# harmoniqs/DirectTrajOpt.jl

Hardware: NVIDIA B200
Metric: full NLP evals/sec (constraint+Jacobian+Hessian) (higher is better)
Workload: dtype f64

## Files before the change

directtrajopt.jl_b200/csrc/bilinear_persistent.cu:

```cuda
#include <stdlib.h>

#include "dto_internal.h"
#include "series_tables.cuh"
#include "bulk_copy.cuh"

namespace {

constexpr int kMaxDrives = 4;
constexpr int kMaxWarps = 12;

__device__ __forceinline__ void dmma(double& c0, double& c1, double a, double b) {
    asm("mma.sync.aligned.m8n8k4.row.col.f64.f64.f64.f64 {%0,%1}, {%2}, {%3}, {%0,%1};" : "+d"(c0), "+d"(c1) : "d"(a), "d"(b));
}

__device__ __forceinline__ double quad_sum(double v) {
    v += __shfl_xor_sync(0xffffffffu, v, 1);
    v += __shfl_xor_sync(0xffffffffu, v, 2);
    return v;
}
__device__ __forceinline__ double warp_max(double v) {
#pragma unroll
    for (int o = 16; o > 0; o >>= 1) v = fmax(v, __shfl_xor_sync(0xffffffffu, v, o));
    return v;
}
// ... 7 lines not shown
template <int MT, int NT, int MD>
__device__ __forceinline__ void mma_apply(double (&out)[MT][NT][2], const double (&v)[MD][NT][2], const double* __restrict__ M,
                                          int lane) {
    constexpr int n = 8 * NT;
    const int row8 = lane >> 2;
    const int d = (NT % 2 == 0) ? ((row8 & 1) << 3) : 0;
    const double* base = M + row8 * n + 2 * (lane & 3);
#pragma unroll
    for (int t = 0; t < NT; ++t) {
        const int off = 8 * t + ((t & 1) ? -d : d);
        double2 b[NT];
#pragma unroll
        for (int nt = 0; nt < NT; ++nt) b[nt] = *reinterpret_cast<const double2*>(base + 8 * nt * n + off);
#pragma unroll
        for (int nt = 0; nt < NT; ++nt)
#pragma unroll
            for (int mt = 0; mt < MT; ++mt) dmma(out[mt][nt][0], out[mt][nt][1], v[mt][t][0], b[nt].x);
#pragma unroll
        for (int nt = 0; nt < NT; ++nt)
#pragma unroll
            for (int mt = 0; mt < MT; ++mt) dmma(out[mt][nt][0], out[mt][nt][1], v[mt][t][1], b[nt].y);
    }
}

template <int MT, int NT>
__device__ __forceinline__ void frag_zero(double (&f)[MT][NT][2]) {
#pragma unroll
    for (int mt = 0; mt < MT; ++mt)
#pragma unroll
        for (int nt = 0; nt < NT; ++nt) f[mt][nt][0] = f[mt][nt][1] = 0.0;
}

enum { ROLE_FWD = 0, ROLE_EXP = 1, ROLE_ADJ = 2 };

template <int NT>
struct Ctx {
    const DProb* P;
    const DInt* I;
    const double* Z;
    const double* mu;
    double* g;
    double* jac;
    const double* Gs;
    double* Gu;
    double* vbuf;
    double* M3;
    double* S2;
    int lane, want_jac, want_hess;
    int jets;
    const double2* plan;
};

template <int NT>
__device__ __forceinline__ double build_generator(const Ctx<NT>& c, const double (&uu)[kMaxDrives], int m, bool need_norm = true) {
    constexpr int n = 8 * NT, nn = n * n;
    for (int p = c.lane; p < nn; p += 32) {
        double v = c.Gs[p];
#pragma unroll
        for (int i = 0; i < kMaxDrives; ++i)
            if (i < m) v = fma(uu[i], c.Gs[(1 + i) * nn + p], v);
        c.Gu[p] = v;
    }
    __syncwarp();
    if (!need_norm) return 0.0;
    double cmax = 0.0;
    for (int k = c.lane; k < n; k += 32) {
        double s1 = 0.0;
        for (int s = 0; s < n; ++s) s1 += fabs(c.Gu[sw<NT>(s, k)]);
        cmax = fmax(cmax, s1);
    }
    return warp_max(cmax);
}

template <int NT>
__device__ __forceinline__ Series interval_series(const Ctx<NT>& c, int b, int kk, double dt, const double (&uu)[kMaxDrives], int m) {
    if (c.plan != nullptr) {
        build_generator<NT>(c, uu, m, false);
        return choose_series(c.plan[(long long)b * c.P->nI + kk]);
    }
    return choose_series(fabs(dt) * build_generator<NT>(c, uu, m));
}

template <int NT>
__device__ __forceinline__ void adjoint_drive_products(const double* __restrict__ Gs, const double* __restrict__ avec,
                                                       double* __restrict__ ybuf, int m, int lane) {
    constexpr int n = 8 * NT, nn = n * n;
    if constexpr (n >= 32) {
        for (int s = lane; s < n; s += 32) {
            double y[kMaxDrives] = {0.0, 0.0, 0.0, 0.0};
            for (int k = 0; k < n; k += 2) {
                const double2 a2 = *reinterpret_cast<const double2*>(avec + k);
                const int p0 = sw<NT>(k, s), p1 = sw<NT>(k + 1, s);
#pragma unroll
                for (int i = 0; i < kMaxDrives; ++i)
                    if (i < m) {
                        y[i] = fma(Gs[(1 + i) * nn + p0], a2.x, y[i]);
                        y[i] = fma(Gs[(1 + i) * nn + p1], a2.y, y[i]);
                    }
            }
#pragma unroll
            for (int i = 0; i < kMaxDrives; ++i)
                if (i < m) ybuf[i * n + s] = y[i];
        }
    } else {
        constexpr int KS = 32 / n;
        constexpr int KL = n / KS;
        const int s = lane % n, part = lane / n;
        double y[kMaxDrives] = {0.0, 0.0, 0.0, 0.0};
        if (part < KS) {
#pragma unroll
            for (int kk = 0; kk < KL; kk += 2) {
                const int k = part * KL + kk;
                const double2 a2 = *reinterpret_cast<const double2*>(avec + k);
                const int p0 = sw<NT>(k, s), p1 = sw<NT>(k + 1, s);
#pragma unroll
                for (int i = 0; i < kMaxDrives; ++i)
                    if (i < m) {
                        y[i] = fma(Gs[(1 + i) * nn + p0], a2.x, y[i]);
                        y[i] = fma(Gs[(1 + i) * nn + p1], a2.y, y[i]);
                    }
            }
        }
#pragma unroll
        for (int i = 0; i < kMaxDrives; ++i)
            if (i < m) {
#pragma unroll
                for (int off = n; off < 32 && off < n * KS; off <<= 1) y[i] += __shfl_xor_sync(0xffffffffu, y[i], off);
                if (lane < n) ybuf[i * n + s] = y[i];
            }
    }
}

template <int NT, int MT>
__device__ __forceinline__ void role_forward(const Ctx<NT>& c, int b, int kk, const int (&src)[kMaxDrives][MT],
                                             const double (&coef)[kMaxDrives][MT]) {
    constexpr int n = 8 * NT, nn = n * n;
    const DProb& P = *c.P;
    const DInt& I = *c.I;
    const int m = I.m, z = P.z, lane = c.lane, q = lane & 3, row8 = lane >> 2;
    const double* zk = c.Z + (long long)b * P.n_vars_local + (long long)kk * z;
    const double* zk1 = zk + z;
    if (P.halo != nullptr && kk + 1 == P.nK - 1) zk1 = P.halo;
    const double dt = zk[P.dt_off];
    double uu[kMaxDrives];
#pragma unroll
    for (int i = 0; i < kMaxDrives; ++i) uu[i] = i < m ? zk[I.u_off + i] : 0.0;
    const Series ser = interval_series<NT>(c, b, kk, dt, uu, m);
    const long long mu_off = (long long)b * P.n_cons_local + I.row_off + (long long)kk * n;
    const bool deriv = c.want_jac || c.want_hess || c.jets == DTO_JETS_STORE;
    const double* Gu = c.Gu;

    double F[MT][NT][2], term[MT][NT][2];
    frag_zero(F);
    if (row8 == 0) {
#pragma unroll
        for (int nt = 0; nt < NT; ++nt) {
            F[0][nt][0] = zk[I.x_off + 8 * nt + 2 * q];
            F[0][nt][1] = zk[I.x_off + 8 * nt + 2 * q + 1];
        }
    }
    for (int st = 0; st < ser.stages; ++st) {
#pragma unroll
        for (int mt = 0; mt < MT; ++mt)
#pragma unroll
            for (int nt = 0; nt < NT; ++nt) {
                term[mt][nt][0] = F[mt][nt][0];
                term[mt][nt][1] = F[mt][nt][1];
            }
        for (int t = 1; t <= ser.terms; ++t) {
            const double cf = dt * ser.inv_stages * kInv[t];
            double nw[MT][NT][2];
            frag_zero(nw);
            mma_apply<MT, NT, MT>(nw, term, Gu, lane);
#pragma unroll
            for (int i = 0; i < kMaxDrives; ++i) {
                if (i < m && deriv) {
                    double tmp[1][NT][2];
                    frag_zero(tmp);
                    mma_apply<1, NT, MT>(tmp, term, c.Gs + (1 + i) * nn, lane);
#pragma unroll
                    for (int mt = 0; mt < MT; ++mt)
#pragma unroll
                        for (int nt = 0; nt < NT; ++nt) {
                            const double v0 = __shfl_sync(0xffffffffu, tmp[0][nt][0], src[i][mt]);
                            const double v1 = __shfl_sync(0xffffffffu, tmp[0][nt][1], src[i][mt]);
                            nw[mt][nt][0] = fma(coef[i][mt], v0, nw[mt][nt][0]);
                            nw[mt][nt][1] = fma(coef[i][mt], v1, nw[mt][nt][1]);
                        }
                }
            }
#pragma unroll
            for (int mt = 0; mt < MT; ++mt)
#pragma unroll
                for (int nt = 0; nt < NT; ++nt) {
                    term[mt][nt][0] = cf * nw[mt][nt][0];
                    term[mt][nt][1] = cf * nw[mt][nt][1];
                    F[mt][nt][0] += term[mt][nt][0];
                    F[mt][nt][1] += term[mt][nt][1];
                }
        }
    }
    double GF[1][NT][2];
    frag_zero(GF);
    mma_apply<1, NT, MT>(GF, F, Gu, lane);
    if (c.g != nullptr && row8 == 0) {
        double* gp = c.g + mu_off;
#pragma unroll
        for (int nt = 0; nt < NT; ++nt) {
            gp[8 * nt + 2 * q] = zk1[I.x_off + 8 * nt + 2 * q] - F[0][nt][0];
            gp[8 * nt + 2 * q + 1] = zk1[I.x_off + 8 * nt + 2 * q + 1] - F[0][nt][1];
        }
    }
    if (c.want_jac) {
        double* jp = c.jac + (long long)b * P.nnz_jac_local;
        const long long own_off = jac_own_off(P, kk, I.doff, n);
        const long long prev_off = jac_prev_off(P, kk + 1, I.doff);
        for (int e = lane; e < 2 * z * n; e += 32) {
            const int l = e / n, a = e % n;
            if (l < z) {
                if ((l >= I.x_off && l < I.x_off + n) || (l >= I.u_off && l < I.u_off + m) || l == P.dt_off) continue;
                jp[jac_col(P, kk, l) + own_off + a] = 0.0;
            } else {
                jp[jac_col(P, (kk + 1), (l - z)) + prev_off + a] = (l - z - I.x_off == a) ? 1.0 : 0.0;
            }
        }
        if (row8 >= 1 && row8 <= m) {
            double* col = jp + jac_col(P, kk, I.u_off + (row8 - 1)) + own_off;
#pragma unroll
            for (int nt = 0; nt < NT; ++nt) {
                col[8 * nt + 2 * q] = -F[0][nt][0];
                col[8 * nt + 2 * q + 1] = -F[0][nt][1];
            }
        }
        if (row8 == 0) {
            double* col = jp + jac_col(P, kk, P.dt_off) + own_off;
#pragma unroll
            for (int nt = 0; nt < NT; ++nt) {
                col[8 * nt + 2 * q] = -GF[0][nt][0];
                col[8 * nt + 2 * q + 1] = -GF[0][nt][1];
            }
        }
    }
    if (c.want_hess && c.jets == DTO_JETS_NONE) {
        const int np = m + 1;
        double* hpp = I.hs + ((long long)b * P.nI + kk) * I.hs_stride + (long long)np * n;
        double muf[NT][2];
#pragma unroll
        for (int nt = 0; nt < NT; ++nt) {
            muf[nt][0] = c.mu[mu_off + 8 * nt + 2 * q];
            muf[nt][1] = c.mu[mu_off + 8 * nt + 2 * q + 1];
        }
#pragma unroll
// ... 62 lines not shown
        double GGF[1][NT][2];
        frag_zero(GGF);
        mma_apply<1, NT, 1>(GGF, GF, Gu, lane);
        if (row8 == 0) {
            double* w = W + (long long)J2 * n;
#pragma unroll
            for (int nt = 0; nt < NT; ++nt) {
                w[8 * nt + 2 * q] = GGF[0][nt][0];
                w[8 * nt + 2 * q + 1] = GGF[0][nt][1];
            }
        }
        if (row8 >= 1 && row8 <= m) {
            double* w = W + (long long)(J2 + 1 + m + (row8 - 1)) * n;
#pragma unroll
            for (int nt = 0; nt < NT; ++nt) {
                w[8 * nt + 2 * q] = GF[0][nt][0];
                w[8 * nt + 2 * q + 1] = GF[0][nt][1];
            }
        }
#pragma unroll
        for (int i = 0; i < kMaxDrives; ++i) {
            if (i < m) {
                double GiF[1][NT][2];
                frag_zero(GiF);
                mma_apply<1, NT, MT>(GiF, F, c.Gs + (1 + i) * nn, lane);
                if (row8 == 0) {
                    double* w = W + (long long)(J2 + 1 + i) * n;
#pragma unroll
                    for (int nt = 0; nt < NT; ++nt) {
                        w[8 * nt + 2 * q] = GiF[0][nt][0];
                        w[8 * nt + 2 * q + 1] = GiF[0][nt][1];
                    }
                }
            }
        }
    }
}

template <int NT, int MT>
__device__ __forceinline__ void role_exp_series(const Ctx<NT>& c, int b, int kk) {
    constexpr int n = 8 * NT;
    const DProb& P = *c.P;
    const DInt& I = *c.I;
    const int m = I.m, z = P.z, lane = c.lane, q = lane & 3, row8 = lane >> 2;
    const double* zk = c.Z + (long long)b * P.n_vars_local + (long long)kk * z;
    const double dt = zk[P.dt_off];
    double uu[kMaxDrives];
#pragma unroll
    for (int i = 0; i < kMaxDrives; ++i) uu[i] = i < m ? zk[I.u_off + i] : 0.0;
    const Series ser = interval_series<NT>(c, b, kk, dt, uu, m);
    double* jp = c.jac + (long long)b * P.nnz_jac_local;
    const long long own_off = jac_own_off(P, kk, I.doff, n);
    for (int c0 = 0; c0 < n; c0 += 8 * MT) {
        double F[MT][NT][2], term[MT][NT][2];
#pragma unroll
        for (int mt = 0; mt < MT; ++mt)
#pragma unroll
            for (int nt = 0; nt < NT; ++nt) {
                const int col = c0 + mt * 8 + row8;
                F[mt][nt][0] = (8 * nt + 2 * q == col) ? 1.0 : 0.0;
                F[mt][nt][1] = (8 * nt + 2 * q + 1 == col) ? 1.0 : 0.0;
            }
        for (int st = 0; st < ser.stages; ++st) {
#pragma unroll
            for (int mt = 0; mt < MT; ++mt)
#pragma unroll
                for (int nt = 0; nt < NT; ++nt) {
                    term[mt][nt][0] = F[mt][nt][0];
                    term[mt][nt][1] = F[mt][nt][1];
                }
            for (int t = 1; t <= ser.terms - 2; ++t) {
                const double cf = dt * ser.inv_stages * kInv[t];
                double nw[MT][NT][2];
                frag_zero(nw);
                mma_apply<MT, NT, MT>(nw, term, c.Gu, lane);
#pragma unroll
                for (int mt = 0; mt < MT; ++mt)
#pragma unroll
                    for (int nt = 0; nt < NT; ++nt) {
                        term[mt][nt][0] = cf * nw[mt][nt][0];
                        term[mt][nt][1] = cf * nw[mt][nt][1];
                        F[mt][nt][0] += term[mt][nt][0];
                        F[mt][nt][1] += term[mt][nt][1];
                    }
            }
        }
#pragma unroll
        for (int mt = 0; mt < MT; ++mt) {
            const int col = c0 + mt * 8 + row8;
            if (col < n) {
                double* cp = jp + jac_col(P, kk, I.x_off + col) + own_off;
#pragma unroll
                for (int nt = 0; nt < NT; ++nt) {
                    cp[8 * nt + 2 * q] = -F[mt][nt][0];
                    cp[8 * nt + 2 * q + 1] = -F[mt][nt][1];
                }
            }
        }
    }
}

template <int NT>
__device__ __forceinline__ void role_exp_ps(const Ctx<NT>& c, int b, int kk) {
    constexpr int n = 8 * NT, nn = n * n;
    constexpr int ME = (NT == 2 || NT == 4) ? 2 : 1;
    constexpr int NCB = NT / ME;
    constexpr int SWZ = (NT % 2 == 0) ? 1 : 0;
    const DProb& P = *c.P;
    const DInt& I = *c.I;
    const int m = I.m, z = P.z, lane = c.lane, q = lane & 3, row8 = lane >> 2;
    const double* zk = c.Z + (long long)b * P.n_vars_local + (long long)kk * z;
    const double dt = zk[P.dt_off];
    double uu[kMaxDrives];
#pragma unroll
    for (int i = 0; i < kMaxDrives; ++i) uu[i] = i < m ? zk[I.u_off + i] : 0.0;
    double theta, alpha;
    if (c.plan != nullptr) {
        build_generator<NT>(c, uu, m, false);
        const double2 pl = c.plan[(long long)b * P.nI + kk];
        alpha = pl.x;
        theta = pl.y;
    } else {
        theta = alpha = fabs(dt) * build_generator<NT>(c, uu, m);
    }
    int sq = 0, nb = 1;
    double scale = dt;
    if (theta < 1e8) {
        double th = theta;
        while (th > 1.5) {
            th *= 0.5;
            alpha *= 0.5;
            scale *= 0.5;
            ++sq;
        }
        nb = (taylor_terms(fmin(th, alpha)) + 2) / 3;
    } else {
        scale = __longlong_as_double(0x7ff8000000000000LL);
// ... 279 lines not shown
    }
}

template <int NT>
constexpr int max_warps() {
    return NT == 1 ? 24 : (NT == 2 ? 16 : kMaxWarps);
}

template <int NT, int MT>
__global__ void __launch_bounds__(max_warps<NT>() * 32, 1)
    bilinear_persistent_kernel(DProb P, int ii, const double* __restrict__ Z, const double* __restrict__ mu, double* __restrict__ g,
                               double* __restrict__ jac, int want_jac, int want_hess, unsigned long long* __restrict__ wq, int nE,
                               int fetch, int jets) {
    extern __shared__ __align__(16) double sm[];
    constexpr int n = 8 * NT, nn = n * n;
    const DInt& I = P.in[ii];
    const int m = I.m;
    const int W = blockDim.x >> 5;
    const int warp = threadIdx.x >> 5, lane = threadIdx.x & 31;
    const int q = lane & 3, row8 = lane >> 2;
    constexpr int slot = nn + (1 + kMaxDrives) * n;

    double* Gs = sm;
    if (I.Gsw != nullptr) {
        __shared__ __align__(8) unsigned long long bar;
        bulk_stage(Gs, I.Gsw, (unsigned)((m + 1) * nn * sizeof(double)), &bar);
    } else {
        for (int e = threadIdx.x; e < (m + 1) * nn; e += blockDim.x) {
            const int i = e / nn, r = e % nn;
            Gs[i * nn + sw<NT>(r / n, r % n)] = I.Grm[e];
        }
        __syncthreads();
    }

    Ctx<NT> c;
    c.P = &P;
    c.I = &I;
    c.Z = Z;
    c.mu = mu;
    c.g = g;
    c.jac = jac;
    c.Gs = Gs;
    c.Gu = Gs + (size_t)(m + 1) * nn + (size_t)warp * slot;
    c.vbuf = c.Gu + nn;
    c.M3 = Gs + (size_t)(m + 1) * nn + (size_t)W * slot + (size_t)warp * 2 * nn;
    c.S2 = c.M3 + nn;
    c.lane = lane;
    c.want_jac = want_jac;
    c.want_hess = want_hess;
    c.jets = jets;
    c.plan = I.plan;
    const bool ps = warp < nE;

    int src[kMaxDrives][MT];
    double coef[kMaxDrives][MT];
#pragma unroll
    for (int mt = 0; mt < MT; ++mt) {
        const int r = mt * 8 + row8;
        int pa = -1, pb = -1;
        if (r >= 1 + m) {
            int p = r - 1 - m, a = 0;
            while (a < m && p >= m - a) {
                p -= m - a;
                ++a;
            }
            if (a < m) {
                pa = a;
                pb = a + p;
            }
        }
#pragma unroll
        for (int i = 0; i < kMaxDrives; ++i) {
            int s_row = 0;
            double cc = 0.0;
            if (i < m) {
                if (r == 1 + i) { s_row = 0; cc = 1.0; }
                else if (pa == i && pb == i) { s_row = 1 + i; cc = 2.0; }
                else if (pa == i) { s_row = 1 + pb; cc = 1.0; }
                else if (pb == i) { s_row = 1 + pa; cc = 1.0; }
            }
            src[i][mt] = s_row * 4 + q;
            coef[i][mt] = cc;
        }
    }

    const int nIc = min(P.kc1, P.nI) - P.kc0;
    const unsigned long long nItems = (unsigned long long)P.batch * (unsigned long long)nIc;
    int order[3];
    int nroles = 0;
    if (ps && want_jac) order[nroles++] = ROLE_EXP;
    if (jets != DTO_JETS_USE) order[nroles++] = ROLE_FWD;
    if (nE == 0 && want_jac) order[nroles++] = ROLE_EXP;
    if (want_hess) order[nroles++] = ROLE_ADJ;
    for (int ri = 0; ri < nroles; ++ri) {
        const int role = order[ri];
        while (true) {
            unsigned long long id0 = 0;
            if (lane == 0) id0 = atomicAdd(&wq[role], (unsigned long long)fetch);
            id0 = __shfl_sync(0xffffffffu, id0, 0);
            if (id0 >= nItems) break;
            for (unsigned long long id = id0; id < id0 + fetch && id < nItems; ++id) {
            const int b = (int)(id / (unsigned long long)nIc), kk = P.kc0 + (int)(id % (unsigned long long)nIc);
            __syncwarp();
#ifndef DTO_SKIP_FWD
            if (role == ROLE_FWD) role_forward<NT, MT>(c, b, kk, src, coef);
#endif
#ifndef DTO_SKIP_ADJ
            if (role == ROLE_ADJ) role_adjoint<NT>(c, b, kk);
#endif
#ifndef DTO_SKIP_PS
            if (role == ROLE_EXP && ps) role_exp_ps<NT>(c, b, kk);
#endif
#ifndef DTO_SKIP_SER
            if (role == ROLE_EXP && !ps) role_exp_series<NT, (NT <= 2 ? 2 : 1)>(c, b, kk);
#endif
            __syncwarp();
            }
        }
    }
    __syncthreads();
    if (threadIdx.x == 0) {
        __threadfence();
        if (atomicAdd(&wq[3], 1ull) == (unsigned long long)gridDim.x - 1) {
            wq[0] = wq[1] = wq[2] = wq[3] = 0ull;
            __threadfence();
        }
    }
}

template <int NT>
__device__ __forceinline__ void product_forward(const Ctx<NT>& c, double* Gw, const double* __restrict__ w, double* __restrict__ y, int b,
                                                int kk) {
    constexpr int n = 8 * NT, nn = n * n;
    const DProb& P = *c.P;
    const DInt& I = *c.I;
    const int m = I.m, z = P.z, lane = c.lane, q = lane & 3, row8 = lane >> 2;
    const double* zk = c.Z + (long long)b * P.n_vars_local + (long long)kk * z;
    const double* wk = w + (long long)b * P.n_vars_local + (long long)kk * z;
    const double dt = zk[P.dt_off], wdt = wk[P.dt_off];
    double uu[kMaxDrives], wu[kMaxDrives];
#pragma unroll
    for (int i = 0; i < kMaxDrives; ++i) {
        uu[i] = i < m ? zk[I.u_off + i] : 0.0;
        wu[i] = i < m ? wk[I.u_off + i] : 0.0;
    }
    const Series ser = choose_series(fabs(dt) * build_generator<NT>(c, uu, m));
    for (int p = lane; p < nn; p += 32) {
        double v = 0.0;
#pragma unroll
        for (int i = 0; i < kMaxDrives; ++i)
            if (i < m) v = fma(wu[i], c.Gs[(1 + i) * nn + p], v);
        Gw[p] = v;
    }
    __syncwarp();
    double F[1][NT][2], term[1][NT][2];
#pragma unroll
    for (int nt = 0; nt < NT; ++nt)
#pragma unroll
// ... 227 lines not shown
    const long long items = (long long)P.batch * P.nI;
    const int grid = (int)std::max<long long>(1, std::min<long long>(sms, (items + W - 1) / W));
    const long long per_warp = items / ((long long)grid * W);
    const int fetch = (NT <= 2) ? (int)std::max<long long>(1, std::min<long long>(8, per_warp / 8)) : 1;
    kern<<<grid, W * 32, smem, st>>>(P, ii, Z, w, y, transpose ? 1 : 0, I.wq, fetch);
    if (cudaMemsetAsync(I.wq, 0, 4 * sizeof(unsigned long long), st) != cudaSuccess) return false;
    ++*launches;
    return true;
}

template <int NT, int MT>
bool launch_variant(const DProb& P, int ii, const double* Z, const double* mu, double* g, double* jac, EvalFlags f, cudaStream_t st,
                    long long* launches) {
    const DInt& I = P.in[ii];
    constexpr int n = 8 * NT;
    const size_t mat = sizeof(double) * (size_t)n * n;
    const size_t slot = mat + sizeof(double) * (1 + kMaxDrives) * n;
    const size_t shared_part = (size_t)(I.m + 1) * mat;
    const size_t budget = 227 * 1024 - 1024;
    if (shared_part + slot > budget) return false;
    int dev = 0, sms = 148;
    cudaGetDevice(&dev);
    cudaDeviceGetAttribute(&sms, cudaDevAttrMultiProcessorCount, dev);
    int W = (int)std::min<size_t>(max_warps<NT>(), (budget - shared_part) / slot);
    int nE = 0;
    if (f.want_jac) {
        int bestW = W, bestE = 0;
        for (int w = W; w >= std::max(2, W - 4); --w) {
            const size_t left = budget - shared_part - (size_t)w * slot;
            const int e = (int)std::min<size_t>((size_t)w, left / (2 * mat));
            if (e >= (w + 2) / 3) {
                bestW = w;
                bestE = std::min(e, (w + 2) / 3);
                break;
            }
            if (e > bestE && w >= W - 2) {
                bestW = w;
                bestE = e;
            }
        }
        W = bestW;
        nE = bestE;
        if (const char* env = getenv("DTO_B200_K1_NE")) nE = std::max(0, std::min(nE, atoi(env)));
    }
    const size_t smem = shared_part + (size_t)W * slot + (size_t)nE * 2 * mat;
    auto kern = bilinear_persistent_kernel<NT, MT>;
    static PerDeviceOnce configured;
    if (configured.first()) {
        if (cudaFuncSetAttribute(kern, cudaFuncAttributeMaxDynamicSharedMemorySize, (int)budget) != cudaSuccess) return false;
    }
    const long long items = (long long)P.batch * (std::min(P.kc1, P.nI) - P.kc0);
    const long long roles = (f.jets != DTO_JETS_USE ? 1 : 0) + (f.want_jac ? 1 : 0) + (f.want_hess ? 1 : 0);
    const long long want_ctas = (items * roles + W - 1) / W;
    const int grid = (int)std::max<long long>(1, std::min<long long>(std::max(1, sms - P.reserve_sms), want_ctas));
    const long long per_warp = items / ((long long)grid * W);
    const int fetch = (NT <= 2) ? (int)std::max<long long>(1, std::min<long long>(8, per_warp / 8)) : 1;
    kern<<<grid, W * 32, smem, st>>>(P, ii, Z, mu, f.want_g ? g : nullptr, jac, f.want_jac ? 1 : 0, f.want_hess ? 1 : 0, I.wq, nE, fetch, f.jets);
    ++*launches;
    return true;
}

}

void bilinear_persistent_swizzled(int n, int m, const double* Grm, double* out) {
    const int NT = n / 8;
    const size_t nn = (size_t)n * n;
    for (int i = 0; i <= m; ++i)
        for (int s = 0; s < n; ++s)
            for (int k = 0; k < n; ++k) out[i * nn + (size_t)s * n + ((NT % 2 == 0) ? (k ^ ((s & 1) << 3)) : k)] = Grm[i * nn + (size_t)s * n + k];
}


bool bilinear_persistent_supported(int n, int m) {
    if (m < 0 || m > kMaxDrives) return false;
    return n == 8 || n == 16 || n == 24 || n == 32 || n == 48 || n == 64;
}

bool launch_bilinear_persistent(const DProb& P, int ii, const double* Z, const double* mu, double* g, double* jac, EvalFlags f,
                                cudaStream_t st, long long* launches) {
    const DInt& I = P.in[ii];
    if (std::min(P.kc1, P.nI) - P.kc0 <= 0) return true;
    if (!bilinear_persistent_supported(I.n, I.m) || I.G_stride != 0 || I.wq == nullptr) return false;
    if (f.jets != DTO_JETS_NONE && I.jets == nullptr) return false;
    const bool second = (f.want_hess && f.jets == DTO_JETS_NONE) || f.jets == DTO_JETS_STORE;
    const int nrows = second ? 1 + I.m + I.m * (I.m + 1) / 2 : 1 + I.m;
    const bool two = nrows > 8;
#define DTO_DISPATCH(NTv)                                                                                      \
    case NTv:                                                                                                  \
        return two ? launch_variant<NTv, 2>(P, ii, Z, mu, g, jac, f, st, launches)                             \
                   : launch_variant<NTv, 1>(P, ii, Z, mu, g, jac, f, st, launches);
    switch (I.n / 8) {
        DTO_DISPATCH(1)
        DTO_DISPATCH(2)
        DTO_DISPATCH(3)
        DTO_DISPATCH(4)
        DTO_DISPATCH(6)
        DTO_DISPATCH(8)
    }
#undef DTO_DISPATCH
    return false;
}

bool launch_bilinear_product(const DProb& P, int ii, const double* Z, const double* w, double* y, bool transpose, cudaStream_t st,
                             long long* launches) {
    const DInt& I = P.in[ii];
    if (P.nI <= 0) return true;
    if (!bilinear_persistent_supported(I.n, I.m) || I.G_stride != 0 || I.wq == nullptr || P.halo != nullptr) return false;
    switch (I.n / 8) {
        case 1: return launch_product_nt<1>(P, ii, Z, w, y, transpose, st, launches);
        case 2: return launch_product_nt<2>(P, ii, Z, w, y, transpose, st, launches);
        case 3: return launch_product_nt<3>(P, ii, Z, w, y, transpose, st, launches);
        case 4: return launch_product_nt<4>(P, ii, Z, w, y, transpose, st, launches);
        case 6: return launch_product_nt<6>(P, ii, Z, w, y, transpose, st, launches);
        case 8: return launch_product_nt<8>(P, ii, Z, w, y, transpose, st, launches);
    }
    return false;
}
```

directtrajopt.jl_b200/csrc/dto_host.cu:

```cuda
#include <math.h>
#include <stdio.h>
#include <stdlib.h>
#include <string.h>

#include <algorithm>
#include <condition_variable>
#include <functional>
#include <limits>
#include <mutex>
#include <new>
#include <thread>

#include "dto_internal.h"
#include "knotfun.cuh"

static thread_local std::string g_create_error;

struct ConEntry {
    long long col_local;
    long long grow;
    long long lrow;
    long long e;
    int ci;
};
// ... 431 lines not shown
    P.n_obj = d->n_objectives;
    P.n_con = d->n_constraints;
    P.n_vars_local = (long long)P.nK * z + G;
    P.n_grad_local = (long long)P.nOwn * z + G;
    P.gl.G = G;

    long long goff = 0, loff = 0;
    int doff = 0;
    for (int i = 0; i < d->n_integrators; ++i) {
        const dto_integrator_desc& s = d->integrators[i];
        h->ints.push_back(s);
        DInt& I = P.in[i];
        I.kind = s.kind;
        I.x_off = s.x_off;
        I.n = s.x_dim;
        I.u_off = s.u_off;
        I.m = s.u_dim;
        I.t_off = s.t_off;
        I.order = s.spline_order;
        I.n_carrier = s.n_carrier;
        I.doff = doff;
        I.row_off = loff;
        I.steps = s.tdb_steps > 0 ? s.tdb_steps : 1;
        if (s.x_dim < 1 || s.x_off < 0 || s.x_off + s.x_dim > z) return fail_create(h, DTO_ERR_INVALID, "integrator state component outside the knot");
        const size_t nn = (size_t)s.x_dim * s.x_dim;
        if (s.kind == DTO_INT_BILINEAR) {
            if (s.u_dim < 0 || s.u_off < 0 || s.u_off + s.u_dim > z || !s.G) return fail_create(h, DTO_ERR_INVALID, "bilinear integrator: bad drive component or missing generators");
            const size_t per = (size_t)(s.u_dim + 1) * nn;
            const size_t cnt = s.G_batch_stride ? (size_t)s.G_batch_stride * (d->batch - 1) + per : per;
            I.G = dev_upload(h, s.G, cnt);
            I.G_stride = s.G_batch_stride;
            {
                std::vector<double> rm(cnt);
                const size_t nmat = cnt / nn;
                for (size_t q = 0; q < nmat; ++q)
                    for (int r = 0; r < s.x_dim; ++r)
                        for (int c = 0; c < s.x_dim; ++c) rm[q * nn + (size_t)r * s.x_dim + c] = s.G[q * nn + (size_t)c * s.x_dim + r];
                I.Grm = dev_upload(h, rm.data(), cnt);
                if (s.G_batch_stride == 0 && s.x_dim % 8 == 0) {
                    std::vector<double> swz(per);
                    bilinear_persistent_swizzled(s.x_dim, s.u_dim, rm.data(), swz.data());
                    I.Gsw = dev_upload(h, swz.data(), per);
                }
            }
            I.hs_stride = (s.u_dim + 1) * s.x_dim + (s.u_dim + 1) * (s.u_dim + 1);
            I.variant = bilinear_dmma_supported(s.x_dim, s.u_dim) ? DTO_VAR_DMMA : DTO_VAR_GENERIC;
            const char* pin = getenv("DTO_B200_KERNEL");
            const bool pin_generic = pin && strcmp(pin, "generic") == 0, pin_dmma = pin && strcmp(pin, "dmma") == 0;
            const bool pin_persistent = pin && strcmp(pin, "persistent") == 0;
            if (bilinear_persistent_supported(s.x_dim, s.u_dim) && s.G_batch_stride == 0 && !pin_dmma && !pin_generic) {
                I.variant = DTO_VAR_PERSISTENT;
                I.wq = dev_upload<unsigned long long>(h, nullptr, 4);
                if (!I.wq) return fail_create(h, DTO_ERR_ALLOC, "device allocation failed (work queue)");
                if (bilinear_octet_supported(s.x_dim, s.u_dim) && !pin_persistent) I.variant = DTO_VAR_OCTET;
            }
            if (s.G_batch_stride != 0 && bilinear_octet_supported(s.x_dim, s.u_dim) && !pin_dmma && !pin_generic && !pin_persistent) {
                const size_t fd = bilinear_octet_fragment_doubles(s.x_dim, s.u_dim);
                std::vector<double> frag(fd * (size_t)d->batch);
                for (int b = 0; b < d->batch; ++b)
                    bilinear_octet_fragments(s.x_dim, s.u_dim, s.G + (size_t)b * s.G_batch_stride, frag.data() + (size_t)b * fd);
                I.bfrag = dev_upload(h, frag.data(), frag.size());
                if (!I.bfrag) return fail_create(h, DTO_ERR_ALLOC, "device allocation failed (generator fragments)");
                I.variant = DTO_VAR_OCTET;
            }
            if (pin_generic) I.variant = DTO_VAR_GENERIC;
            if (s.x_dim > 96) return fail_create(h, DTO_ERR_UNSUPPORTED, "bilinear integrator: state dimension > 96 not supported");
            if (I.variant == DTO_VAR_GENERIC) {
                const size_t need = generic_smem_bytes(s.x_dim, s.u_dim, true, d->eval_hessian);
                if (need > (size_t)smem_optin)
                    return fail_create(h, DTO_ERR_UNSUPPORTED, smem_msg("bilinear integrator: the generic kernel at state dimension " +
                                                                        std::to_string(s.x_dim) + " with " + std::to_string(s.u_dim) +
                                                                        " drives" + (d->eval_hessian ? " and the Hessian" : ""), need));
            }
        } else if (s.kind == DTO_INT_DERIVATIVE) {
            if (s.u_dim != s.x_dim || s.u_off < 0 || s.u_off + s.u_dim > z) return fail_create(h, DTO_ERR_INVALID, "derivative integrator: derivative component must match the variable's dimension");
        } else if (s.kind == DTO_INT_TDBILINEAR) {
            if (s.u_dim < 0 || s.u_off < 0 || s.u_off + s.u_dim > z || s.t_off < 0 || s.t_off >= z || !s.G)
                return fail_create(h, DTO_ERR_INVALID, "tdbilinear integrator: bad components");
            if (!tdb_available()) return fail_create(h, DTO_ERR_UNSUPPORTED, "tdbilinear integrator kernel is not built into this library");
            if (s.spline_order != 0 && s.spline_order != 1) return fail_create(h, DTO_ERR_UNSUPPORTED, "Unsupported spline order");
            I.G = dev_upload(h, s.G, nn);
            I.A = dev_upload(h, s.A, nn * s.u_dim);
            I.B = dev_upload(h, s.B, nn * s.u_dim);
            I.omega = dev_upload(h, s.omega, s.u_dim);
            I.phi = dev_upload(h, s.phi, s.u_dim);
            I.D = dev_upload(h, s.D, nn * s.n_carrier);
            I.omega_d = dev_upload(h, s.omega_d, s.n_carrier);
            I.phi_d = dev_upload(h, s.phi_d, s.n_carrier);
            {
                auto norm1 = [&](const double* M) {
                    double best = 0.0;
                    for (int c = 0; c < s.x_dim; ++c) {
                        double sum = 0.0;
                        for (int r = 0; r < s.x_dim; ++r) sum += fabs(M[(size_t)c * s.x_dim + r]);
                        best = std::max(best, sum);
                    }
                    return best;
                };
                std::vector<double> bn((size_t)std::max(s.u_dim, 1), 0.0);
                I.tdb_gnorm = norm1(s.G);
                I.tdb_wmax = 0.0;
                {
                    const char* tl = getenv("DTO_B200_TDB_TOL");
                    I.tdb_tol = tl ? atof(tl) : 1e-14;
                }
                for (int i = 0; i < s.u_dim; ++i) {
// ... 1788 lines not shown
```

directtrajopt.jl_b200/csrc/dto_internal.h:

```cpp
#pragma once
#include <cuda_runtime.h>
#include <stdint.h>

#include <algorithm>
#include <string>
#include <vector>

#include "../../include/dto_b200.h"

#define DTO_MAX_INT 8
#define DTO_MAX_OBJ 16
#define DTO_MAX_CON 8
#define DTO_MAX_KNOTFN_VARS 128

enum { DTO_OP_OUT = 16 };
struct DProgram {
    const int4* code;
    int n_code;
    int _pad;
    __host__ __device__ const double* consts() const { return reinterpret_cast<const double*>(code + n_code); }
};
struct DInt {
    int kind, x_off, n, u_off, m, t_off, order, n_carrier;
    int doff;
    int hs_stride;
    int steps;
    double tdb_gnorm;
    double tdb_wmax;
    double tdb_tol;
    const double* tdb_bnorm;
    int variant;
    long long row_off;
    long long G_stride;
    const double* G;
    const double* Grm;
    const double* bfrag;
    const double *A, *B, *omega, *phi, *D, *omega_d, *phi_d;
    const double *Asw, *Bsw, *Dsw;
    double* tdb_scratch;
    int tdb_scratch_ctas;
    double* hs;
    double* jets;
    int jet_stride;
    const double2* plan;
    const double* Gsw;
    const float* planmat;
    unsigned long long* wq;
};

struct DObj {
    int kind, fn;
    double weight;
    int nv, nt, np;
    int nvk;
    double D;
    const int* var_offs;
    const int* g2l;
    const int* own_ti;
    const int* own_knot;
    int nt_own;
    int own_kmin, own_kmax;
    const int* knot_to_own;
    long long side_off;
    const double* R;
    const double* baseline;
    const double* params;
    const double* Qs;
    DProgram prog;
};

struct DCon {
    int fn, nv, nt_own, gd, np;
    int nvk;
    long long row_off;
    const int* var_offs;
    const int* g2l;
    const int* own_ti;
    const int* own_knot;
    const int* knot_to_own;
    const double* params;
    const long long* jac_pos;
    DProgram prog;
};

struct DGlob {
    int G;
    int S, S_obj;
    int KV;
    const int* slot_term;
    const int* slot_j;
    const long long* kg_pos;
    const long long* gg_pos;
    double* scratchG;
    double* scratchH;
    long long hess_tail_off;
    long long n_hess_tail;
};

struct DProb {
    int N;
// ... 83 lines not shown
    unsigned long long hs_seq;
    unsigned long long hs_ack;
    unsigned long long pad;
    double scal[2][DTO_MAX_RANKS][4];
    double halo[2];
};
struct HsRows {
    double* row[DTO_MAX_INT];
    int len[DTO_MAX_INT];
    int n;
};
__host__ __device__ inline double* xwin_hblk(XWin* w, int z) { return w->halo + 2 * (size_t)z; }
void launch_shard_publish(XWin* own, XWin* left, XWin* right, double* dst, const double* src, long long n, int z,
                          unsigned long long epoch, bool wait_right, cudaStream_t st, long long* launches);
void launch_shard_wait(XWin* own, unsigned long long epoch, cudaStream_t st, long long* launches);
void launch_hs_push(XWin* own, XWin* right, const HsRows& rows, int z, long long hblk_len, unsigned long long seq, cudaStream_t st,
                    long long* launches);
void launch_hs_receive(XWin* own, XWin* left, const HsRows& rows, int z, long long hblk_len, unsigned long long seq, cudaStream_t st,
                       long long* launches);
void launch_scalar_exchange(XWin* own, XWin* const* peers, int rank, int world, unsigned long long seq, double* J, double* viol,
                            cudaStream_t st, long long* launches);

void launch_shard_scalars(XWin* own, XWin* const* peers, int rank, int world, unsigned long long seq, long long n_cons, const double* g,
                          const int* row_is_eq, unsigned long long* scratch, double* J, double* viol, cudaStream_t st, long long* launches);

enum { DTO_VAR_GENERIC = 0, DTO_VAR_DMMA = 1, DTO_VAR_PERSISTENT = 2, DTO_VAR_OCTET = 3 };

struct PerDeviceOnce {
    bool done[64] = {};
    bool first() {
        int d = 0;
        if (cudaGetDevice(&d) != cudaSuccess || d < 0 || d >= 64) return true;
        if (done[d]) return false;
        done[d] = true;
        return true;
    }
};

enum { DTO_JETS_NONE = 0, DTO_JETS_STORE = 1, DTO_JETS_USE = 2 };
struct EvalFlags {
    bool want_g, want_jac, want_hess;
    int jets = DTO_JETS_NONE;
};
void launch_hpp_contract(const DProb& P, int ii, const double* mu, cudaStream_t st, long long* launches);
void launch_bilinear_generic(const DProb& P, int ii, const double* Z, const double* mu, double* g, double* jac, EvalFlags f,
                             cudaStream_t st, long long* launches);
size_t generic_smem_bytes(int n, int m, bool want_jac, bool want_hess);
bool launch_bilinear_dmma(const DProb& P, int ii, const double* Z, const double* mu, double* g, double* jac, EvalFlags f,
                          cudaStream_t st, long long* launches);
bool bilinear_dmma_supported(int n, int m);
bool launch_bilinear_persistent(const DProb& P, int ii, const double* Z, const double* mu, double* g, double* jac, EvalFlags f,
                                cudaStream_t st, long long* launches);
bool bilinear_persistent_supported(int n, int m);
bool launch_bilinear_octet(const DProb& P, int ii, const double* Z, const double* mu, double* g, double* jac, EvalFlags f,
                           cudaStream_t st, long long* launches);
bool bilinear_octet_supported(int n, int m);
void bilinear_octet_fragments(int n, int m, const double* Gcm, double* out);
size_t bilinear_octet_fragment_doubles(int n, int m);
bool launch_bilinear_product(const DProb& P, int ii, const double* Z, const double* w, double* y, bool transpose, cudaStream_t st,
                             long long* launches);
void launch_analytic_product(const DProb& P, const double* Z, const double* w, double* y, bool transpose, cudaStream_t st,
                             long long* launches);
void bilinear_persistent_swizzled(int n, int m, const double* Grm, double* out);
size_t series_plan_smem(int n, int m);
void series_plan_matrices(int n, int m, const double* Gcm, std::vector<float>& out);
bool launch_series_plan(const DProb& P, int ii, const double* Z, cudaStream_t st, long long* launches);
bool tdb_available();
bool tdb_dmma_supported(const DInt& I);
bool launch_tdb_dmma(const DProb& P, int ii, const double* Z, const double* mu, double* g, double* jac, EvalFlags f, cudaStream_t st,
                     long long* launches);
bool tdb_fits(const DInt& I, size_t smem_limit);
void launch_tdb(const DProb& P, int ii, const double* Z, const double* mu, double* g, double* jac, EvalFlags f, cudaStream_t st,
                long long* launches);
void launch_analytic(const DProb& P, const double* Z, double* g, double* jac, EvalFlags f, cudaStream_t st, long long* launches);
void launch_constraints(const DProb& P, const double* Z, double* g, double* jac, EvalFlags f, cudaStream_t st, long long* launches);
bool launch_knot_objective_pairs(const DProb& P, const double* Z, cudaStream_t st, long long* launches);
void launch_hessian_assemble(const DProb& P, const double* Z, double sigma, const double* mu, double* hess, cudaStream_t st,
                             long long* launches, bool left_block = false);
size_t hessian_assemble_smem_bytes(const DProb& P);
void launch_objective(const DProb& P, const double* Z, double* J, double* grad, double* partials, cudaStream_t st,
                      long long* launches);
void launch_violation(const DProb& P, const double* g, const int* row_is_eq, double* viol, cudaStream_t st, long long* launches);
void launch_global_gradient(const DProb& P, const double* Z, double* grad, cudaStream_t st, long long* launches);
void launch_global_hessian(const DProb& P, const double* Z, double sigma, const double* mu, double* hess, double* kg_probe,
                           cudaStream_t st, long long* launches);
void launch_jac_product(const DProb& P, const double* jac, const long long* rows0, const long long* cols0, const double* w,
                        double* y, bool transpose, cudaStream_t st, long long* launches);
void launch_knot_program(const DProb& P, int ci, const double* Z, double* g, double* jac, double* dense_probe, cudaStream_t st,
                         long long* launches);
void launch_constraint_pattern_probe(const DProb& P, const double* Z, double* dense_jac , cudaStream_t st,
                                     long long* launches);
```

Before: 3573.

## Evaluate exponential series by Horner form and spill stage start to scratch

The forward and exponential-series roles now evaluate the truncated Taylor series in Horner form. This removes the separate `term` fragment array. The per-stage starting value is written to a per-warp global scratch slot and read back in each fused multiply-add, instead of being held in registers. Per-drive shuffle source and coefficient tables are packed into one unsigned word per fragment row, the role ordering loop is simplified, and the grid is clamped to the number of CTAs the new scratch buffer was sized for. The aim is lower register pressure and better occupancy, at the cost of extra global/L1 memory traffic in the inner loop.

```diff
diff --git a/directtrajopt.jl_b200/csrc/bilinear_persistent.cu b/directtrajopt.jl_b200/csrc/bilinear_persistent.cu
--- a/directtrajopt.jl_b200/csrc/bilinear_persistent.cu
+++ b/directtrajopt.jl_b200/csrc/bilinear_persistent.cu
@@ -83,6 +83,12 @@
 };
 
 template <int NT>
+__device__ __forceinline__ double* stage_slot(const Ctx<NT>& c) {
+    const int warps = blockDim.x >> 5, warp = threadIdx.x >> 5;
+    return c.I->fwd_stage + ((size_t)blockIdx.x * warps + warp) * (2 * NT * 2 * 32) + c.lane;
+}
+
+template <int NT>
 __device__ __forceinline__ double build_generator(const Ctx<NT>& c, const double (&uu)[kMaxDrives], int m, bool need_norm = true) {
     constexpr int n = 8 * NT, nn = n * n;
     for (int p = c.lane; p < nn; p += 32) {
@@ -163,8 +169,7 @@
 }
 
 template <int NT, int MT>
-__device__ __forceinline__ void role_forward(const Ctx<NT>& c, int b, int kk, const int (&src)[kMaxDrives][MT],
-                                             const double (&coef)[kMaxDrives][MT]) {
+__device__ __forceinline__ void role_forward(const Ctx<NT>& c, int b, int kk, const unsigned (&route)[MT]) {
     constexpr int n = 8 * NT, nn = n * n;
     const DProb& P = *c.P;
     const DInt& I = *c.I;
@@ -181,7 +186,7 @@
     const bool deriv = c.want_jac || c.want_hess || c.jets == DTO_JETS_STORE;
     const double* Gu = c.Gu;
 
-    double F[MT][NT][2], term[MT][NT][2];
+    double F[MT][NT][2];
     frag_zero(F);
     if (row8 == 0) {
 #pragma unroll
@@ -191,44 +196,61 @@
         }
     }
     for (int st = 0; st < ser.stages; ++st) {
-#pragma unroll
-        for (int mt = 0; mt < MT; ++mt)
-#pragma unroll
-            for (int nt = 0; nt < NT; ++nt) {
-                term[mt][nt][0] = F[mt][nt][0];
-                term[mt][nt][1] = F[mt][nt][1];
-            }
-        for (int t = 1; t <= ser.terms; ++t) {
+        if (st > 0) {
+#pragma unroll
+            for (int mt = 0; mt < MT; ++mt)
+#pragma unroll
+                for (int nt = 0; nt < NT; ++nt) {
+                    stage_slot(c)[((mt * NT + nt) * 2 + 0) * 32] = F[mt][nt][0];
+                    stage_slot(c)[((mt * NT + nt) * 2 + 1) * 32] = F[mt][nt][1];
+                }
+        }
+        for (int t = ser.terms; t >= 1; --t) {
             const double cf = dt * ser.inv_stages * kInv[t];
             double nw[MT][NT][2];
             frag_zero(nw);
-            mma_apply<MT, NT, MT>(nw, term, Gu, lane);
+#pragma unroll
+            for (int mt = MT - 1; mt >= 0; --mt)
+                mma_apply<1, NT, 1>(reinterpret_cast<double (&)[1][NT][2]>(nw[mt]), reinterpret_cast<const double (&)[1][NT][2]>(F[mt]), Gu, lane);
 #pragma unroll
             for (int i = 0; i < kMaxDrives; ++i) {
                 if (i < m && deriv) {
                     double tmp[1][NT][2];
                     frag_zero(tmp);
-                    mma_apply<1, NT, MT>(tmp, term, c.Gs + (1 + i) * nn, lane);
-#pragma unroll
-                    for (int mt = 0; mt < MT; ++mt)
+                    mma_apply<1, NT, MT>(tmp, F, c.Gs + (1 + i) * nn, lane);
+#pragma unroll
+                    for (int mt = 0; mt < MT; ++mt) {
+                        const unsigned e = (route[mt] >> (8 * i)) & 0xffu;
+                        const int src = (int)(e & 31u);
+                        const unsigned k = e >> 5;
+                        const double cc = __hiloint2double(k ? (int)(0x3ff00000u + ((k - 1u) << 20)) : 0, 0);
 #pragma unroll
                         for (int nt = 0; nt < NT; ++nt) {
-                            const double v0 = __shfl_sync(0xffffffffu, tmp[0][nt][0], src[i][mt]);
-                            const double v1 = __shfl_sync(0xffffffffu, tmp[0][nt][1], src[i][mt]);
-                            nw[mt][nt][0] = fma(coef[i][mt], v0, nw[mt][nt][0]);
-                            nw[mt][nt][1] = fma(coef[i][mt], v1, nw[mt][nt][1]);
+                            const double v0 = __shfl_sync(0xffffffffu, tmp[0][nt][0], src);
+                            const double v1 = __shfl_sync(0xffffffffu, tmp[0][nt][1], src);
+                            nw[mt][nt][0] = fma(cc, v0, nw[mt][nt][0]);
+                            nw[mt][nt][1] = fma(cc, v1, nw[mt][nt][1]);
                         }
-                }
-            }
-#pragma unroll
-            for (int mt = 0; mt < MT; ++mt)
-#pragma unroll
-                for (int nt = 0; nt < NT; ++nt) {
-                    term[mt][nt][0] = cf * nw[mt][nt][0];
-                    term[mt][nt][1] = cf * nw[mt][nt][1];
-                    F[mt][nt][0] += term[mt][nt][0];
-                    F[mt][nt][1] += term[mt][nt][1];
-                }
+                    }
+                }
+            }
+            asm volatile("" ::: "memory");
+            if (st == 0) {
+#pragma unroll
+                for (int mt = 0; mt < MT; ++mt)
+#pragma unroll
+                    for (int nt = 0; nt < NT; ++nt)
+#pragma unroll
+                        for (int j = 0; j < 2; ++j)
+                            F[mt][nt][j] = (mt == 0 && row8 == 0) ? fma(cf, nw[mt][nt][j], zk[I.x_off + 8 * nt + 2 * q + j]) : cf * nw[mt][nt][j];
+            } else {
+#pragma unroll
+                for (int mt = 0; mt < MT; ++mt)
+#pragma unroll
+                    for (int nt = 0; nt < NT; ++nt)
+#pragma unroll
+                        for (int j = 0; j < 2; ++j) F[mt][nt][j] = fma(cf, nw[mt][nt][j], stage_slot(c)[((mt * NT + nt) * 2 + j) * 32]);
+            }
         }
     }
     double GF[1][NT][2];
@@ -397,37 +419,39 @@
     double* jp = c.jac + (long long)b * P.nnz_jac_local;
     const long long own_off = jac_own_off(P, kk, I.doff, n);
     for (int c0 = 0; c0 < n; c0 += 8 * MT) {
-        double F[MT][NT][2], term[MT][NT][2];
+        double F[MT][NT][2];
 #pragma unroll
         for (int mt = 0; mt < MT; ++mt)
 #pragma unroll
-            for (int nt = 0; nt < NT; ++nt) {
-                const int col = c0 + mt * 8 + row8;
-                F[mt][nt][0] = (8 * nt + 2 * q == col) ? 1.0 : 0.0;
-                F[mt][nt][1] = (8 * nt + 2 * q + 1 == col) ? 1.0 : 0.0;
-            }
+            for (int nt = 0; nt < NT; ++nt)
+#pragma unroll
+                for (int j = 0; j < 2; ++j) F[mt][nt][j] = (8 * nt + 2 * q + j == c0 + mt * 8 + row8) ? 1.0 : 0.0;
         for (int st = 0; st < ser.stages; ++st) {
-#pragma unroll
-            for (int mt = 0; mt < MT; ++mt)
-#pragma unroll
-                for (int nt = 0; nt < NT; ++nt) {
-                    term[mt][nt][0] = F[mt][nt][0];
-                    term[mt][nt][1] = F[mt][nt][1];
-                }
-            for (int t = 1; t <= ser.terms - 2; ++t) {
+            if (st > 0) {
+#pragma unroll
+                for (int mt = 0; mt < MT; ++mt)
+#pragma unroll
+                    for (int nt = 0; nt < NT; ++nt) {
+                        stage_slot(c)[((mt * NT + nt) * 2 + 0) * 32] = F[mt][nt][0];
+                        stage_slot(c)[((mt * NT + nt) * 2 + 1) * 32] = F[mt][nt][1];
+                    }
+            }
+            for (int t = ser.terms - 2; t >= 1; --t) {
                 const double cf = dt * ser.inv_stages * kInv[t];
                 double nw[MT][NT][2];
                 frag_zero(nw);
-                mma_apply<MT, NT, MT>(nw, term, c.Gu, lane);
+                mma_apply<MT, NT, MT>(nw, F, c.Gu, lane);
+                asm volatile("" ::: "memory");
 #pragma unroll
                 for (int mt = 0; mt < MT; ++mt)
 #pragma unroll
-                    for (int nt = 0; nt < NT; ++nt) {
-                        term[mt][nt][0] = cf * nw[mt][nt][0];
-                        term[mt][nt][1] = cf * nw[mt][nt][1];
-                        F[mt][nt][0] += term[mt][nt][0];
-                        F[mt][nt][1] += term[mt][nt][1];
-                    }
+                    for (int nt = 0; nt < NT; ++nt)
+#pragma unroll
+                        for (int j = 0; j < 2; ++j) {
+                            const double v = st == 0 ? ((8 * nt + 2 * q + j == c0 + mt * 8 + row8) ? 1.0 : 0.0)
+                                                     : stage_slot(c)[((mt * NT + nt) * 2 + j) * 32];
+                            F[mt][nt][j] = fma(cf, nw[mt][nt][j], v);
+                        }
             }
         }
 #pragma unroll
@@ -813,8 +837,7 @@
     c.plan = I.plan;
     const bool ps = warp < nE;
 
-    int src[kMaxDrives][MT];
-    double coef[kMaxDrives][MT];
+    unsigned route[MT];
 #pragma unroll
     for (int mt = 0; mt < MT; ++mt) {
         const int r = mt * 8 + row8;
@@ -830,31 +853,27 @@
                 pb = a + p;
             }
         }
+        route[mt] = 0u;
 #pragma unroll
         for (int i = 0; i < kMaxDrives; ++i) {
-            int s_row = 0;
-            double cc = 0.0;
+            unsigned s_row = 0u, cc = 0u;
             if (i < m) {
-                if (r == 1 + i) { s_row = 0; cc = 1.0; }
-                else if (pa == i && pb == i) { s_row = 1 + i; cc = 2.0; }
-                else if (pa == i) { s_row = 1 + pb; cc = 1.0; }
-                else if (pb == i) { s_row = 1 + pa; cc = 1.0; }
-            }
-            src[i][mt] = s_row * 4 + q;
-            coef[i][mt] = cc;
+                if (r == 1 + i) { s_row = 0u; cc = 1u; }
+                else if (pa == i && pb == i) { s_row = 1u + i; cc = 2u; }
+                else if (pa == i) { s_row = 1u + pb; cc = 1u; }
+                else if (pb == i) { s_row = 1u + pa; cc = 1u; }
+            }
+            route[mt] |= (s_row * 4u + q | cc << 5) << (8 * i);
         }
     }
 
     const int nIc = min(P.kc1, P.nI) - P.kc0;
     const unsigned long long nItems = (unsigned long long)P.batch * (unsigned long long)nIc;
-    int order[3];
-    int nroles = 0;
-    if (ps && want_jac) order[nroles++] = ROLE_EXP;
-    if (jets != DTO_JETS_USE) order[nroles++] = ROLE_FWD;
-    if (nE == 0 && want_jac) order[nroles++] = ROLE_EXP;
-    if (want_hess) order[nroles++] = ROLE_ADJ;
-    for (int ri = 0; ri < nroles; ++ri) {
-        const int role = order[ri];
+    for (int k = 0; k < 3; ++k) {
+        const int role = (ps && k < 2) ? (k == 0 ? ROLE_EXP : ROLE_FWD) : k;
+        if (role == ROLE_FWD && jets == DTO_JETS_USE) continue;
+        if (role == ROLE_EXP && !(want_jac && (ps || nE == 0))) continue;
+        if (role == ROLE_ADJ && !want_hess) continue;
         while (true) {
             unsigned long long id0 = 0;
             if (lane == 0) id0 = atomicAdd(&wq[role], (unsigned long long)fetch);
@@ -864,7 +883,7 @@
             const int b = (int)(id / (unsigned long long)nIc), kk = P.kc0 + (int)(id % (unsigned long long)nIc);
             __syncwarp();
 #ifndef DTO_SKIP_FWD
-            if (role == ROLE_FWD) role_forward<NT, MT>(c, b, kk, src, coef);
+            if (role == ROLE_FWD) role_forward<NT, MT>(c, b, kk, route);
 #endif
 #ifndef DTO_SKIP_ADJ
             if (role == ROLE_ADJ) role_adjoint<NT>(c, b, kk);
@@ -1198,7 +1217,7 @@
     const long long items = (long long)P.batch * (std::min(P.kc1, P.nI) - P.kc0);
     const long long roles = (f.jets != DTO_JETS_USE ? 1 : 0) + (f.want_jac ? 1 : 0) + (f.want_hess ? 1 : 0);
     const long long want_ctas = (items * roles + W - 1) / W;
-    const int grid = (int)std::max<long long>(1, std::min<long long>(std::max(1, sms - P.reserve_sms), want_ctas));
+    const int grid = (int)std::max<long long>(1, std::min<long long>(std::min(I.fwd_stage_ctas, std::max(1, sms - P.reserve_sms)), want_ctas));
     const long long per_warp = items / ((long long)grid * W);
     const int fetch = (NT <= 2) ? (int)std::max<long long>(1, std::min<long long>(8, per_warp / 8)) : 1;
     kern<<<grid, W * 32, smem, st>>>(P, ii, Z, mu, f.want_g ? g : nullptr, jac, f.want_jac ? 1 : 0, f.want_hess ? 1 : 0, I.wq, nE, fetch, f.jets);
@@ -1216,6 +1235,11 @@
             for (int k = 0; k < n; ++k) out[i * nn + (size_t)s * n + ((NT % 2 == 0) ? (k ^ ((s & 1) << 3)) : k)] = Grm[i * nn + (size_t)s * n + k];
 }
 
+
+size_t bilinear_persistent_stage_doubles(int n, int ctas) {
+    const int W = n == 8 ? max_warps<1>() : n == 16 ? max_warps<2>() : max_warps<3>();
+    return (size_t)ctas * W * 2 * 8 * n;
+}
 
 bool bilinear_persistent_supported(int n, int m) {
     if (m < 0 || m > kMaxDrives) return false;
diff --git a/directtrajopt.jl_b200/csrc/dto_host.cu b/directtrajopt.jl_b200/csrc/dto_host.cu
--- a/directtrajopt.jl_b200/csrc/dto_host.cu
+++ b/directtrajopt.jl_b200/csrc/dto_host.cu
@@ -507,6 +507,11 @@
                 I.variant = DTO_VAR_PERSISTENT;
                 I.wq = dev_upload<unsigned long long>(h, nullptr, 4);
                 if (!I.wq) return fail_create(h, DTO_ERR_ALLOC, "device allocation failed (work queue)");
+                int sms = 148;
+                cudaDeviceGetAttribute(&sms, cudaDevAttrMultiProcessorCount, h->device);
+                I.fwd_stage_ctas = sms;
+                I.fwd_stage = dev_upload<double>(h, nullptr, bilinear_persistent_stage_doubles(s.x_dim, sms));
+                if (!I.fwd_stage) return fail_create(h, DTO_ERR_ALLOC, "device allocation failed (forward stage buffer)");
                 if (bilinear_octet_supported(s.x_dim, s.u_dim) && !pin_persistent) I.variant = DTO_VAR_OCTET;
             }
             if (s.G_batch_stride != 0 && bilinear_octet_supported(s.x_dim, s.u_dim) && !pin_dmma && !pin_generic && !pin_persistent) {
diff --git a/directtrajopt.jl_b200/csrc/dto_internal.h b/directtrajopt.jl_b200/csrc/dto_internal.h
--- a/directtrajopt.jl_b200/csrc/dto_internal.h
+++ b/directtrajopt.jl_b200/csrc/dto_internal.h
@@ -46,6 +46,8 @@
     const double* Gsw;
     const float* planmat;
     unsigned long long* wq;
+    double* fwd_stage;
+    int fwd_stage_ctas;
 };
 
 struct DObj {
@@ -235,6 +237,7 @@
 bool launch_bilinear_persistent(const DProb& P, int ii, const double* Z, const double* mu, double* g, double* jac, EvalFlags f,
                                 cudaStream_t st, long long* launches);
 bool bilinear_persistent_supported(int n, int m);
+size_t bilinear_persistent_stage_doubles(int n, int ctas);
 bool launch_bilinear_octet(const DProb& P, int ii, const double* Z, const double* mu, double* g, double* jac, EvalFlags f,
                            cudaStream_t st, long long* launches);
 bool bilinear_octet_supported(int n, int m);
```

Result: no change. 3600, median of 6 (+0.8%).
